# lifunudt/CORB-SLAM

Measured on AMD Instinct MI355X. Metric: stereo frames/sec ORB extract+match, higher is better.
Workload: dtype u8; 1 GPU; configs[1]: ORB extract+match, synthetic 1241x376 stereo stream, 2000 feat/frame, 8 levels x1.2, FAST 20/7; warmup_frames_per_gpu=2560, batches_in_flight=1, distinct_frames=64, parallelism=1 client per GPU, replicas (no collective), inputs=resident in HBM

## Files before the change

### corb-slam_amd/csrc/corb_internal.h

```cpp
#pragma once
#include <hip/hip_runtime.h>
#include <stdint.h>
#include <stddef.h>
#include "../../include/corb_accel.h"

#include <stdlib.h>
#ifdef CORB_DEV
static inline const char* corb_dev_env(const char* name) { return getenv(name); }
#else
static inline const char* corb_dev_env(const char*) { return nullptr; }
#endif

#define CORB_MAX_LEVELS 16
#define CORB_EDGE_THRESHOLD 19
#define CORB_MIN_BORDER 16
#define CORB_HALF_PATCH 15
#define CORB_PATCH_SIZE 31
#define CORB_TH_HIGH 100
#define CORB_TH_LOW 50
#define CORB_HISTO_LENGTH 30

struct CorbLevel {
    int w, h, pitch;
    int plane_off;
    int nCols, nRows, wCell, hCell;
    int maxBX, maxBY;
    int cell_base;
    int cell_cap;
    int cand_base;
    int cand_cap;
    int quota;
    int kp_base, kp_cap;
    int nIni;
    int node_cap;
    int blur_tile_base, blur_tiles_x, blur_tiles_y;
    int resize_tab_off;
    int resize_rec_off;
    float scale;
    float hX;
    int patch_size;
};

#define CORB_BLUR_T 64
#define CORB_MAX_PARTS 4

struct CorbOrbParams {
    int nlevels, n_images;
    int img_base;
    int ini_th, min_th;
    int cells_per_image, cand_per_image, kp_per_image, out_cap;
    int blur_tiles_per_image;
    int node_cap_max, ncell_max;
    int fast_tp, fast_th;
    int pyr_strips;
    short pyr_r0[8][CORB_MAX_LEVELS], pyr_r1[8][CORB_MAX_LEVELS];
    int pyr_ctiles;
    short pyr_g0[8][CORB_MAX_LEVELS], pyr_g1[8][CORB_MAX_LEVELS];
    size_t arena_per_image;
    uint8_t* pyr;
    uint8_t* blur;
    int* cell_count;
    uint32_t* cand;
    uint32_t* keys;
    uint16_t* key_node;
    uint32_t* kp;
    int* kp_count;
    const short* resize_tab;
    const int2* resize_rec;
    CorbKeyPoint* out_kp;
    uint8_t* out_desc;
    int* out_count;
    int* status;
    CorbLevel lv[CORB_MAX_LEVELS];
};

struct CorbStereoParams {
    int n_frames, nlevels;
    int frame_base;
    float bf, mb;
    float scale[CORB_MAX_LEVELS], inv_scale[CORB_MAX_LEVELS];
    int rows0;
    float* u_right;
    float* depth;
    int* sad;
    int* n_matched;
    int* row_off;
    int2* row_idx;
    int row_cap;
    int2* left_range;
};

#ifdef __HIPCC__
__device__ __forceinline__ void corb_xcd_remap(int& unit, int& img)
{
    const unsigned nx = gridDim.x, nimg = gridDim.y;
    const unsigned B = blockIdx.x + nx * blockIdx.y;
    const unsigned g = B / (8u * nx), r = B - g * 8u * nx;
    const unsigned in_group = min(8u, nimg - 8u * g);
    img = (int)(8u * g + r % in_group);
    unit = (int)(r / in_group);
}
#endif

struct CorbStereoDeviceFrame { const CorbKeyPoint* kp; const uint8_t* desc; const float* u_right; const float* depth; const int* count; int cap; hipStream_t stream; int device; };
struct CorbStereo;
int corb_stereo_device_frame(CorbStereo* h, int frame, CorbStereoDeviceFrame* out);
struct CorbRgbd;
int corb_rgbd_device_frame(CorbRgbd* h, int frame, CorbStereoDeviceFrame* out);

struct CorbProfiler;
void corb_orb_device_init();
void corb_launch_ingest(const uint8_t* stage, int w, int h, int n_images, uint8_t* plane, int pitch, size_t image_stride, hipStream_t stream);
void corb_launch_stereo_pack(const CorbOrbParams& p, const CorbStereoParams& s, int frame_base, int n_frames, uint8_t* out, const CorbStereoFrameLayout& lay, hipStream_t stream, struct CorbProfiler* prof);
void corb_launch_orb_pipeline(const CorbOrbParams& p, int img_base, int n_images, size_t octree_lds, hipStream_t stream, CorbProfiler* prof, hipEvent_t after_fast = nullptr);
void corb_launch_candidates(const CorbOrbParams* dp, int img, int level, CorbKeyPoint* out, int cap, int* n_out, hipStream_t stream);
void corb_launch_stereo(const CorbOrbParams& p, const CorbStereoParams& s, int frame_base, int n_frames, hipStream_t stream, CorbProfiler* prof);
size_t corb_octree_lds_bytes(int node_cap_max, int ncell_max);

#ifdef __HIPCC__
#include <hip/hip_ext.h>
#define CORB_LAUNCH(prof, name, kernel, grid, block, lds, stream, ...) do { \
    if ((prof) && (prof)->enabled) { hipEvent_t ea_, eb_; (prof)->pair(name, &ea_, &eb_); hipExtLaunchKernelGGL(kernel, grid, block, (std::uint32_t)(lds), stream, ea_, eb_, 0, __VA_ARGS__); } \
    else hipLaunchKernelGGL(kernel, grid, block, lds, stream, __VA_ARGS__); } while (0)
#endif
#include <vector>
#include <string>
struct CorbProfiler {
    bool enabled = false;
    bool serial = false;
    struct Rec { int name_id; hipEvent_t a, b; };
    std::vector<std::string> names;
    std::vector<Rec> recs;
    std::vector<hipEvent_t> pool;
    int name_id(const char* n) { for (size_t i = 0; i < names.size(); i++) if (names[i] == n) return (int)i; names.push_back(n); return (int)names.size() - 1; }
    void reserve(size_t n) { while (pool.size() < n) { hipEvent_t e; if (hipEventCreate(&e) != hipSuccess) break; pool.push_back(e); } }
    hipEvent_t get() { if (!pool.empty()) { hipEvent_t e = pool.back(); pool.pop_back(); return e; } hipEvent_t e; (void)hipEventCreate(&e); return e; }
    void pair(const char* n, hipEvent_t* a, hipEvent_t* b) { Rec r; r.name_id = name_id(n); r.a = get(); r.b = get(); recs.push_back(r); *a = r.a; *b = r.b; }
    ~CorbProfiler() { for (auto& r : recs) { (void)hipEventDestroy(r.a); (void)hipEventDestroy(r.b); } for (auto e : pool) (void)hipEventDestroy(e); }
};
```

### corb-slam_amd/csrc/corb_orb.cpp

```cpp
#include "corb_internal.h"
#include "orb_handle.h"
#include <cmath>
#include <cfloat>
#include <cstdio>
#include <cstdarg>
#include <cstring>
#include <mutex>
#include <map>
#include <vector>

static thread_local char g_err[512] = "";
void corb_set_error(const char* fmt, ...)
{
    va_list ap; va_start(ap, fmt); vsnprintf(g_err, sizeof(g_err), fmt, ap); va_end(ap);
}
extern "C" const char* corb_last_error(void) { return g_err; }
extern "C" int corb_version(void) { return 100; }
extern "C" int corb_abi_version(void) { return CORB_ABI_VERSION; }
extern "C" int corb_device_count(void)
{
    int n = 0;
    if (hipGetDeviceCount(&n) != hipSuccess) return 0;
    return n;
}
// ... 67 lines not shown
extern "C" int corb_orb_create(const CorbOrbConfig* cfg, CorbOrb** out)
{
    if (!cfg || !out) { corb_set_error("null argument"); return CORB_ERR_ARG; }
    *out = nullptr;
    if (cfg->nlevels < 1 || cfg->nlevels > CORB_MAX_LEVELS || cfg->nfeatures < 1 || cfg->max_images < 1 ||
        cfg->width < 1 || cfg->height < 1 || cfg->width > 4000 || cfg->height > 4000 || !(cfg->scale_factor > 1.0f) ||
        cfg->min_th_fast < 1 || cfg->ini_th_fast < cfg->min_th_fast || cfg->ini_th_fast > 255) {
        corb_set_error("invalid CorbOrbConfig"); return CORB_ERR_ARG;
    }
    int rc = corb_select_device(cfg->device);
    if (rc != CORB_OK) return rc;
    CorbOrb* h = new CorbOrb();
    h->cfg = *cfg;
    const int nl = cfg->nlevels;
    h->scale[0] = 1.0f; h->sigma2[0] = 1.0f;
    for (int i = 1; i < nl; i++) { h->scale[i] = h->scale[i - 1] * cfg->scale_factor; h->sigma2[i] = h->scale[i] * h->scale[i]; }
    for (int i = 0; i < nl; i++) { h->inv_scale[i] = 1.0f / h->scale[i]; h->inv_sigma2[i] = 1.0f / h->sigma2[i]; }
    {
        float factor = 1.0f / cfg->scale_factor;
        float nDesired = cfg->nfeatures * (1 - factor) / (1 - (float)pow((double)factor, (double)nl));
        int sum = 0;
        for (int level = 0; level < nl - 1; level++) { h->quota[level] = cv_round(nDesired); sum += h->quota[level]; nDesired *= factor; }
        h->quota[nl - 1] = std::max(cfg->nfeatures - sum, 0);
        int v, v0, vmax = cv_floor(CORB_HALF_PATCH * sqrtf(2.f) / 2 + 1), vmin = cv_ceil(CORB_HALF_PATCH * sqrtf(2.f) / 2);
        const double hp2 = CORB_HALF_PATCH * CORB_HALF_PATCH;
        for (v = 0; v <= vmax; ++v) h->umax[v] = cv_round(sqrt(hp2 - v * v));
        for (v = CORB_HALF_PATCH, v0 = 0; v >= vmin; --v) { while (h->umax[v0] == h->umax[v0 + 1]) ++v0; h->umax[v] = v0; ++v0; }
        static const int expect[16] = {15, 15, 15, 15, 14, 14, 14, 13, 13, 12, 11, 10, 9, 8, 6, 3};
        for (int i = 0; i < 16; i++) if (h->umax[i] != expect[i]) { corb_set_error("umax table mismatch"); delete h; return CORB_ERR_ARG; }
    }
    CorbOrbParams& p = h->p;
    memset(&p, 0, sizeof(p));
    p.nlevels = nl; p.n_images = cfg->max_images; p.ini_th = cfg->ini_th_fast; p.min_th = cfg->min_th_fast;
    size_t arena = 0; int cells = 0, cands = 0, kps = 0, tiles = 0, tab_off = 0, rec_off = 0;
    for (int l = 0; l < nl; l++) {
        CorbLevel& L = p.lv[l];
        L.w = cv_round((float)cfg->width * h->inv_scale[l]);
        L.h = cv_round((float)cfg->height * h->inv_scale[l]);
        L.pitch = (L.w + 63) & ~63;
        L.plane_off = (int)arena;
        arena += ((size_t)L.pitch * L.h + 255) & ~(size_t)255;
        L.maxBX = L.w - CORB_EDGE_THRESHOLD + 3; L.maxBY = L.h - CORB_EDGE_THRESHOLD + 3;
        const float width = (float)(L.maxBX - CORB_MIN_BORDER), height = (float)(L.maxBY - CORB_MIN_BORDER);
        L.nCols = (int)(width / 30.f); L.nRows = (int)(height / 30.f);
        if (L.nCols < 1 || L.nRows < 1) { corb_set_error("level %d (%dx%d) too small for the 30-px FAST grid", l, L.w, L.h); delete h; return CORB_ERR_ARG; }
        L.wCell = (int)ceilf(width / L.nCols); L.hCell = (int)ceilf(height / L.nRows);
        if (L.wCell > 64 || L.hCell > 64) { corb_set_error("FAST cell %dx%d exceeds the LDS tile", L.wCell, L.hCell); delete h; return CORB_ERR_ARG; }
        L.cell_base = cells; cells += L.nCols * L.nRows;
        L.cell_cap = ((L.wCell + 1) / 2) * ((L.hCell + 1) / 2);
        L.cand_base = cands; L.cand_cap = L.nCols * L.nRows * L.cell_cap; cands += L.cand_cap;
        L.quota = h->quota[l];
        int nIni = (int)roundf(width / height);
        if (nIni < 1) nIni = 1;
        L.nIni = nIni;
        L.hX = width / nIni;
        L.node_cap = ((std::max(L.quota + 3, 4 * nIni) + 1) + 3) & ~3;
        L.kp_base = kps; L.kp_cap = L.node_cap; kps += L.kp_cap;
        L.blur_tiles_x = (L.w + 3) / 4; L.blur_tiles_y = (L.h + 31) / 32;
        L.blur_tile_base = tiles; tiles += (L.blur_tiles_x * L.blur_tiles_y + CORB_BLUR_T - 1) / CORB_BLUR_T;
        L.resize_tab_off = tab_off; tab_off += 3 * L.w + 4 * L.h;
        L.resize_rec_off = rec_off; rec_off += ((L.w + 3) & ~3) + L.h + 4;
        L.scale = h->scale[l];
        L.patch_size = (int)(CORB_PATCH_SIZE * h->scale[l]);
        p.node_cap_max = std::max(p.node_cap_max, L.node_cap);
        p.ncell_max = std::max(p.ncell_max, L.nCols * L.nRows);
        p.fast_tp = std::max(p.fast_tp, 4 * ((L.wCell + 3) / 4) + 8);
        p.fast_th = std::max(p.fast_th, L.hCell + 6);
    }
    p.cells_per_image = cells; p.cand_per_image = cands; p.kp_per_image = kps; p.out_cap = kps;
    p.blur_tiles_per_image = tiles; p.arena_per_image = arena;
    h->octree_lds = corb_octree_lds_bytes(p.node_cap_max, p.ncell_max);
    if (h->octree_lds > 160 * 1024) { corb_set_error("quadtree needs %zu B of LDS (> 160 KiB): nfeatures too large", h->octree_lds); delete h; return CORB_ERR_ARG; }
    if (p.node_cap_max > 65535) { corb_set_error("nfeatures too large"); delete h; return CORB_ERR_ARG; }
    const size_t NI = (size_t)cfg->max_images;
    short* d_tab = nullptr;
#define DA(ptr, n) do { rc = dalloc(h, &(ptr), (n)); if (rc != CORB_OK) { corb_orb_destroy(h); return rc; } } while (0)
    DA(p.pyr, NI * arena); DA(p.blur, NI * arena);
    DA(p.cell_count, NI * cells); DA(p.cand, NI * cands); DA(p.keys, NI * cands); DA(p.key_node, NI * cands);
    DA(p.kp, NI * kps); DA(p.kp_count, NI * CORB_MAX_LEVELS);
    DA(p.out_kp, NI * p.out_cap); DA(p.out_desc, NI * p.out_cap * 32); DA(p.out_count, NI); DA(p.status, NI);
    DA(d_tab, (size_t)tab_off);
    int2* d_rec = nullptr;
    DA(d_rec, (size_t)rec_off + 4);
    DA(h->dp, 1);
#undef DA
    p.resize_tab = d_tab;
    p.resize_rec = d_rec;
    {
        std::vector<short> tab(tab_off);
        for (int l = 1; l < nl; l++) build_resize_tables(p.lv[l - 1].w, p.lv[l - 1].h, p.lv[l].w, p.lv[l].h, tab.data() + p.lv[l].resize_tab_off);
        std::vector<int2> rec((size_t)rec_off + 4, make_int2(0, 0));
        for (int l = 1; l < nl; l++) {
            const short* tl = tab.data() + p.lv[l].resize_tab_off; const int w = p.lv[l].w, hh = p.lv[l].h;
            int2* xr = rec.data() + p.lv[l].resize_rec_off; int2* yr = xr + ((w + 3) & ~3);
            for (int x = 0; x < ((w + 3) & ~3); x++) { const int xc = std::min(x, w - 1); xr[x] = make_int2(tl[xc], (int)(unsigned short)tl[w + xc] | ((int)(unsigned short)tl[2 * w + xc] << 16)); }
            const short* ys0 = tl + 3 * w; const short* ys1 = ys0 + hh; const short* yb0 = ys1 + hh; const short* yb1 = yb0 + hh;
            for (int y = 0; y < hh; y++) yr[y] = make_int2((int)(unsigned short)ys0[y] | ((int)(unsigned short)ys1[y] << 16), (int)(unsigned short)yb0[y] | ((int)(unsigned short)yb1[y] << 16));
        }
        if (hipMemcpy(d_rec, rec.data(), rec.size() * sizeof(int2), hipMemcpyHostToDevice) != hipSuccess) { corb_set_error("resize record upload failed"); corb_orb_destroy(h); return CORB_ERR_HIP; }
        const int S = 4;
        p.pyr_strips = (nl > 1 && p.lv[nl - 1].h >= 4 * S) ? S : 0;
        for (int s = 0; s < p.pyr_strips; s++) {
            int lo = 0, hi = 0;
            for (int l = nl - 1; l >= 1; l--) {
                const int blo = (int)((long long)s * p.lv[l].h / S), bhi = (int)((long long)(s + 1) * p.lv[l].h / S);
                if (l == nl - 1) { lo = blo; hi = bhi; }
                else {
                    const short* tl = tab.data() + p.lv[l + 1].resize_tab_off;
                    const short* ys0 = tl + 3 * p.lv[l + 1].w; const short* ys1 = ys0 + p.lv[l + 1].h;
                    const int clo = ys0[lo], chi = ys1[hi - 1] + 1;
                    lo = std::min(blo, clo); hi = std::max(bhi, chi);
                }
                p.pyr_r0[s][l] = (short)lo; p.pyr_r1[s][l] = (short)hi;
            }
        }
        const int C = 4;
        p.pyr_ctiles = (p.pyr_strips > 0 && p.lv[nl - 1].w >= 16 * C) ? C : 1;
        for (int c = 0; c < p.pyr_ctiles; c++) {
            int lo = 0, hi = 0;
            for (int l = nl - 1; l >= 1; l--) {
                const int ng = (p.lv[l].w + 3) / 4;
                const int blo = (int)((long long)c * ng / p.pyr_ctiles), bhi = (int)((long long)(c + 1) * ng / p.pyr_ctiles);
                if (l == nl - 1) { lo = blo; hi = bhi; }
                else {
                    const short* xofs = tab.data() + p.lv[l + 1].resize_tab_off;
                    const int wn = p.lv[l + 1].w, x_first = std::min(4 * lo, wn - 1), x_last = std::min(4 * hi, wn) - 1;
                    const int clo = xofs[x_first] / 4, chi = std::min(xofs[x_last] + 1, p.lv[l].w - 1) / 4 + 1;
                    lo = std::min(blo, clo); hi = std::max(bhi, chi);
                }
                p.pyr_g0[c][l] = (short)lo; p.pyr_g1[c][l] = (short)hi;
            }
        }
        if (hipMemcpy(d_tab, tab.data(), tab.size() * sizeof(short), hipMemcpyHostToDevice) != hipSuccess ||
            hipMemcpy(h->dp, &p, sizeof(p), hipMemcpyHostToDevice) != hipSuccess ||
            hipMemset(p.status, 0, NI * sizeof(int)) != hipSuccess || hipMemset(p.out_count, 0, NI * sizeof(int)) != hipSuccess ||
            hipMemset(p.pyr, 0, NI * arena) != hipSuccess || hipMemset(p.blur, 0, NI * arena) != hipSuccess ||
            hipStreamCreateWithFlags(&h->stream, hipStreamNonBlocking) != hipSuccess ||
            hipHostMalloc((void**)&h->h_status, NI * sizeof(int)) != hipSuccess ||
            hipHostMalloc((void**)&h->h_count, NI * sizeof(int)) != hipSuccess ||
            hipMalloc((void**)&h->d_stage, (size_t)cfg->width * cfg->height + 256) != hipSuccess ||
            hipHostMalloc((void**)&h->h_img, (size_t)cfg->width * cfg->height) != hipSuccess ||
            hipHostMalloc((void**)&h->h_kp, (size_t)p.out_cap * sizeof(CorbKeyPoint)) != hipSuccess ||
            hipHostMalloc((void**)&h->h_desc, (size_t)p.out_cap * 32) != hipSuccess ||
            hipHostMalloc((void**)&h->h_f32, (size_t)p.out_cap * 2 * sizeof(float)) != hipSuccess ||
            hipHostMalloc((void**)&h->h_misc, 8 * sizeof(int)) != hipSuccess) {
            corb_set_error("device initialisation failed: %s", hipGetErrorString(hipGetLastError()));
            corb_orb_destroy(h); return CORB_ERR_HIP;
        }
    }
    if (const char* e = getenv("CORB_PARTS")) h->parts = std::max(1, std::min(CORB_MAX_PARTS, atoi(e)));
    for (int i = 0; i < CORB_MAX_PARTS; i++)
        if (hipEventCreateWithFlags(&h->ev_stage[i], hipEventDisableTiming) != hipSuccess) { corb_set_error("event creation failed: %s", hipGetErrorString(hipGetLastError())); corb_orb_destroy(h); return CORB_ERR_HIP; }
    *out = h;
    return CORB_OK;
}

extern "C" void corb_orb_destroy(CorbOrb* h)
{
    if (!h) return;
    (void)hipSetDevice(h->cfg.device);
    if (h->stream) { (void)hipStreamSynchronize(h->stream); (void)hipStreamDestroy(h->stream); }
    for (int i = 0; i < CORB_MAX_PARTS - 1; i++) {
        if (h->side[i]) { (void)hipStreamSynchronize(h->side[i]); (void)hipStreamDestroy(h->side[i]); }
        if (h->ev_done[i]) (void)hipEventDestroy(h->ev_done[i]);
    }
    for (int i = 0; i < CORB_MAX_PARTS; i++) if (h->ev_stage[i]) (void)hipEventDestroy(h->ev_stage[i]);
    for (void* ptr : h->allocs) (void)hipFree(ptr);
    if (h->h_status) (void)hipHostFree(h->h_status);
    if (h->h_count) (void)hipHostFree(h->h_count);
    if (h->d_stage) (void)hipFree(h->d_stage);
// ... 448 lines not shown
```

### corb-slam_amd/csrc/orb_kernels.hip

```cpp
#include "corb_internal.h"
#include "lane_exchange.h"
#include <atomic>
#include <cstring>
#include <cstdlib>
#include "brief_pattern.h"

#define WAVE 64

struct CorbDescribeTab { uint4 patb[64]; };
__device__ CorbDescribeTab g_dsc_tab;


#define RS_ROWS 8
__global__ __launch_bounds__(256) void orb_resize_kernel(const CorbOrbParams p, int level)
{
    const CorbLevel& D = p.lv[level];
    const CorbLevel& S = p.lv[level - 1];
    const int img = p.img_base + blockIdx.z;
    const int x4 = (blockIdx.x * 64 + threadIdx.x) * 4;
    const int yb = (blockIdx.y * 4 + threadIdx.y) * RS_ROWS;
    if (x4 >= D.w || yb >= D.h) return;
    const short* tab = p.resize_tab + D.resize_tab_off;
    const short* xofs = tab, * xa0 = tab + D.w, * xa1 = tab + 2 * D.w;
    const short* ys0 = tab + 3 * D.w, * ys1 = ys0 + D.h, * yb0 = ys1 + D.h, * yb1 = yb0 + D.h;
// ... 105 lines not shown
                s1b |= (uint32_t)(ob < 8 ? ob : 0x0c) << (8 * k); s2b |= (uint32_t)(ob < 8 ? k : ob - 4) << (8 * k);
            }
            const bool patch_a = __any(wide && sx[3] - bx >= 8), patch_b = __any(wide && sx1[3] - bx >= 8);
            if (wide) {
                auto fetch = [&](const int2 yr, uint32_t (&w)[6], uint32_t& bb) {
                    const uint32_t* q0 = reinterpret_cast<const uint32_t*>(src + (uint32_t)(__mul24(yr.x & 0xFFFF, S.pitch) + bx));
                    const uint32_t* q1 = reinterpret_cast<const uint32_t*>(src + (uint32_t)(__mul24(yr.x >> 16, S.pitch) + bx));
                    w[0] = q0[0]; w[1] = q0[1]; w[2] = q0[2]; w[3] = q1[0]; w[4] = q1[1]; w[5] = q1[2];
                    bb = (uint32_t)yr.y;
                };
                auto emit = [&](int y, const uint32_t (&w)[6], uint32_t bb) {
                    const uint32_t b0 = bb & 0xFFFFu, b1 = bb >> 16;
                    uint32_t P0 = __builtin_amdgcn_perm(w[1], w[0], s1a), P1 = __builtin_amdgcn_perm(w[1], w[0], s1b);
                    uint32_t Q0 = __builtin_amdgcn_perm(w[4], w[3], s1a), Q1 = __builtin_amdgcn_perm(w[4], w[3], s1b);
                    if (patch_a) { P0 = __builtin_amdgcn_perm(w[2], P0, s2a); Q0 = __builtin_amdgcn_perm(w[5], Q0, s2a); }
                    if (patch_b) { P1 = __builtin_amdgcn_perm(w[2], P1, s2b); Q1 = __builtin_amdgcn_perm(w[5], Q1, s2b); }
                    uint32_t packed = 0;
                    pyr_px<0>(packed, P0, P1, Q0, Q1, A0[0], A1[0], b0, b1, two);
                    pyr_px<1>(packed, P0, P1, Q0, Q1, A0[1], A1[1], b0, b1, two);
                    pyr_px<2>(packed, P0, P1, Q0, Q1, A0[2], A1[2], b0, b1, two);
                    pyr_px<3>(packed, P0, P1, Q0, Q1, A0[3], A1[3], b0, b1, two);
                    uint8_t* dst = dstp + (uint32_t)(__mul24(y, D.pitch) + x4);
                    if (nvalid == 4) *reinterpret_cast<uint32_t*>(dst) = packed;
                    else for (int k = 0; k < nvalid; k++) dst[k] = (uint8_t)(packed >> (8 * k));
                };
                int y = r0 + ty;
                const int ylast = max(r1 - 1, 0);
                int2 ya = yrec[min(y, ylast)], yb = yrec[min(y + RY, ylast)];
                int2 yc = yrec[min(y + 2 * RY, ylast)], yd = yrec[min(y + 3 * RY, ylast)];
#pragma unroll 1
                for (; y + 3 * RY < r1; y += 4 * RY) {
                    uint32_t wa[6], wb[6], wc[6], wd[6], ba, bb, bc, bd;
                    fetch(ya, wa, ba); fetch(yb, wb, bb); fetch(yc, wc, bc); fetch(yd, wd, bd);
                    const int2 na = yrec[min(y + 4 * RY, ylast)], nb = yrec[min(y + 5 * RY, ylast)], nc = yrec[min(y + 6 * RY, ylast)], nd = yrec[min(y + 7 * RY, ylast)];
                    emit(y, wa, ba); emit(y + RY, wb, bb); emit(y + 2 * RY, wc, bc); emit(y + 3 * RY, wd, bd);
                    ya = na; yb = nb; yc = nc; yd = nd;
                }
                if (y + RY < r1) {
                    uint32_t wa[6], wb[6], ba, bb;
                    fetch(ya, wa, ba); fetch(yb, wb, bb);
                    emit(y, wa, ba); emit(y + RY, wb, bb);
                    y += 2 * RY; ya = yc; yb = yd;
                }
                if (y < r1) { uint32_t wa[6], ba; fetch(ya, wa, ba); emit(y, wa, ba); }
            } else {
#pragma unroll 1
                for (int y = r0 + ty; y < r1; y += RY) {
                    const int2 yr = yrec[y];
                    const uint8_t* S0 = src + (uint32_t)__mul24(yr.x & 0xFFFF, S.pitch);
                    const uint8_t* S1 = src + (uint32_t)__mul24(yr.x >> 16, S.pitch);
                    const uint32_t b0 = yr.y & 0xFFFF, b1 = (uint32_t)yr.y >> 16;
                    uint32_t packed = 0;
#pragma unroll
                    for (int k = 0; k < 4; k++) {
                        const uint32_t d0 = mad24u(S0[sx[k]], A0[k] >> 12, mul24u(S0[sx1[k]], A1[k] >> 12));
                        const uint32_t d1 = mad24u(S1[sx[k]], A0[k] >> 12, mul24u(S1[sx1[k]], A1[k] >> 12));
                        const uint32_t v = (((mul24u(b0, d0 >> 4) >> 16) + (mul24u(b1, d1 >> 4) >> 16) + 2u) >> 2) & 0xFFu;
                        packed |= v << (8 * k);
                    }
                    uint8_t* dst = dstp + (uint32_t)(__mul24(y, D.pitch) + x4);
                    if (nvalid == 4) *reinterpret_cast<uint32_t*>(dst) = packed;
                    else for (int k = 0; k < nvalid; k++) dst[k] = (uint8_t)(packed >> (8 * k));
                }
            }
        }
        __threadfence_block();
        __syncthreads();
    }
}


__device__ __forceinline__ uint32_t pk_min3(uint32_t a, uint32_t b, uint32_t c)
{ uint32_t d; asm("v_pk_minimum3_f16 %0, %1, %2, %3" : "=v"(d) : "v"(a), "v"(b), "v"(c)); return d; }
__device__ __forceinline__ uint32_t pk_max3(uint32_t a, uint32_t b, uint32_t c)
{ uint32_t d; asm("v_pk_maximum3_f16 %0, %1, %2, %3" : "=v"(d) : "v"(a), "v"(b), "v"(c)); return d; }
template <int K> __device__ __forceinline__ uint32_t pk_pair(const uint32_t (&w)[3])
{
    static_assert(K >= 0 && K <= 10, "window");
    if constexpr (K <= 6) return __builtin_amdgcn_perm(w[1], w[0], 0x0c000c00u | (uint32_t)K | ((uint32_t)(K + 1) << 16));
    else return __builtin_amdgcn_perm(w[2], w[1], 0x0c000c00u | (uint32_t)(K - 4) | ((uint32_t)(K - 3) << 16));
}
typedef short corb_short2 __attribute__((ext_vector_type(2)));

__device__ __forceinline__ uint32_t fast_ring_score(const uint32_t (&v)[16], uint32_t cpk)
{
    uint32_t lo3[16], hi3[16];
#pragma unroll
    for (int i = 0; i < 16; i++) {
        lo3[i] = pk_min3(v[i], v[(i + 1) & 15], v[(i + 2) & 15]);
        hi3[i] = pk_max3(v[i], v[(i + 1) & 15], v[(i + 2) & 15]);
    }
    uint32_t lo9[16], hi9[16];
#pragma unroll
    for (int i = 0; i < 16; i++) {
        lo9[i] = pk_min3(lo3[i], lo3[(i + 3) & 15], lo3[(i + 6) & 15]);
        hi9[i] = pk_max3(hi3[i], hi3[(i + 3) & 15], hi3[(i + 6) & 15]);
    }
    uint32_t b5[5], d5[5];
#pragma unroll
    for (int i = 0; i < 5; i++) { b5[i] = pk_max3(lo9[3 * i], lo9[3 * i + 1], lo9[3 * i + 2]); d5[i] = pk_min3(hi9[3 * i], hi9[3 * i + 1], hi9[3 * i + 2]); }
    const uint32_t B = pk_max3(pk_max3(b5[0], b5[1], b5[2]), pk_max3(b5[3], b5[4], lo9[15]), b5[0]);
    const uint32_t D = pk_min3(pk_min3(d5[0], d5[1], d5[2]), pk_min3(d5[3], d5[4], hi9[15]), d5[0]);
    const corb_short2 c = __builtin_bit_cast(corb_short2, cpk);
    const corb_short2 s = __builtin_elementwise_max(__builtin_bit_cast(corb_short2, B) - c, c - __builtin_bit_cast(corb_short2, D)) - (short)1;
    return __builtin_bit_cast(uint32_t, s);
}

template <int J> __device__ __forceinline__ uint32_t fast_pair_score(const uint32_t (&R)[7][3], uint32_t th2)
{
    constexpr int C = 4 + 2 * J;
    uint32_t v[16];
    v[0] = pk_pair<C>(R[6]);      v[1] = pk_pair<C + 1>(R[6]);  v[2] = pk_pair<C + 2>(R[5]);  v[3] = pk_pair<C + 3>(R[4]);
    v[4] = pk_pair<C + 3>(R[3]);  v[5] = pk_pair<C + 3>(R[2]);  v[6] = pk_pair<C + 2>(R[1]);  v[7] = pk_pair<C + 1>(R[0]);
    v[8] = pk_pair<C>(R[0]);      v[9] = pk_pair<C - 1>(R[0]);  v[10] = pk_pair<C - 2>(R[1]); v[11] = pk_pair<C - 3>(R[2]);
    v[12] = pk_pair<C - 3>(R[3]); v[13] = pk_pair<C - 3>(R[4]); v[14] = pk_pair<C - 2>(R[5]); v[15] = pk_pair<C - 1>(R[6]);
    const corb_short2 s = __builtin_bit_cast(corb_short2, fast_ring_score(v, pk_pair<C>(R[3])));
    const corb_short2 keep = s >= __builtin_bit_cast(corb_short2, th2);
    return __builtin_bit_cast(uint32_t, (corb_short2)(s & keep));
}

template <int J> __device__ __forceinline__ uint32_t fast_compass(const uint32_t (&R0)[3], const uint32_t (&R3)[3], const uint32_t (&R6)[3])
{
    constexpr int C = 4 + 2 * J;
    const uint32_t v0 = pk_pair<C>(R6), v4 = pk_pair<C + 3>(R3), v8 = pk_pair<C>(R0), v12 = pk_pair<C - 3>(R3), cpk = pk_pair<C>(R3);
    const uint32_t m = pk_min3(pk_max3(v0, v8, v8), pk_max3(v4, v12, v12), pk_max3(v4, v12, v12));
    const uint32_t n = pk_max3(pk_min3(v0, v8, v8), pk_min3(v4, v12, v12), pk_min3(v4, v12, v12));
    const corb_short2 c = __builtin_bit_cast(corb_short2, cpk);
    return __builtin_bit_cast(uint32_t, __builtin_elementwise_max(__builtin_bit_cast(corb_short2, m) - c, c - __builtin_bit_cast(corb_short2, n)));
}
__device__ __forceinline__ int mbcnt64(unsigned long long m) { return (int)__builtin_amdgcn_mbcnt_hi((uint32_t)(m >> 32), __builtin_amdgcn_mbcnt_lo((uint32_t)m, 0u)); }

#define FAST_LIST_CAP 512
__device__ __forceinline__ int wave_incl_scan(int v)
{
    v += __builtin_amdgcn_update_dpp(0, v, 0x111, 0xf, 0xf, true);
    v += __builtin_amdgcn_update_dpp(0, v, 0x112, 0xf, 0xf, true);
    v += __builtin_amdgcn_update_dpp(0, v, 0x114, 0xf, 0xf, true);
    v += __builtin_amdgcn_update_dpp(0, v, 0x118, 0xf, 0xf, true);
    v += __builtin_amdgcn_update_dpp(0, v, 0x142, 0xa, 0xf, true);
    v += __builtin_amdgcn_update_dpp(0, v, 0x143, 0xc, 0xf, true);
    return v;
}
template <int TP>
__global__ __launch_bounds__(64) void orb_fast_kernel(const CorbOrbParams p)
{
    constexpr int P = TP / 4;
    extern __shared__ __attribute__((aligned(16))) uint8_t fast_smem[];
    __shared__ uint16_t plist[FAST_LIST_CAP];
    uint32_t* tile = reinterpret_cast<uint32_t*>(fast_smem);
    uint32_t* sc = tile + P * p.fast_th;
    uint32_t (*rowm)[2] = reinterpret_cast<uint32_t (*)[2]>(sc + P * p.fast_th);
    const int nrowm = p.fast_th - 6;
    uint8_t* scb = reinterpret_cast<uint8_t*>(sc);
    int cell, img; corb_xcd_remap(cell, img); img += p.img_base;
    const int lane = threadIdx.x;
    int level = 0;
    for (int l = 1; l < p.nlevels; l++) if (cell >= p.lv[l].cell_base) level = l;
    const CorbLevel& L = p.lv[level];
    const int c = cell - L.cell_base;
    const int ci = c / L.nCols, cj = c - ci * L.nCols;
    const int iniX = CORB_MIN_BORDER + cj * L.wCell, iniY = CORB_MIN_BORDER + ci * L.hCell;
    const int maxX = min(iniX + L.wCell + 6, L.maxBX), maxY = min(iniY + L.hCell + 6, L.maxBY);
    const int cw = maxX - iniX, ch = maxY - iniY;
    int* out_count = p.cell_count + (size_t)img * p.cells_per_image + cell;
    if (cw < 7 || ch < 7) { if (lane == 0) *out_count = 0; return; }
    const int iw = cw - 6, ih = ch - 6;
    {
        const int gx0 = iniX - 1, a = gx0 & 3;
        const uint8_t* src = p.pyr + (size_t)img * p.arena_per_image + L.plane_off + (size_t)iniY * L.pitch + (gx0 - a);
        const int jlast = (a + cw) >> 2;
        const int r0 = lane / P, wc = lane - r0 * P;
        constexpr int RPI = 64 / P;
        if (r0 < RPI) {
            const int j0 = min(wc, jlast), j1 = min(wc + 1, jlast);
            for (int y = r0; y < ch; y += 4 * RPI) {
                uint32_t w0[4], w1[4];
#pragma unroll
                for (int k = 0; k < 4; k++) {
                    const uint32_t* g = reinterpret_cast<const uint32_t*>(src + (uint32_t)__mul24(min(y + k * RPI, ch - 1), L.pitch));
                    w0[k] = g[j0]; w1[k] = g[j1];
                }
#pragma unroll
                for (int k = 0; k < 4; k++)
                    if (y + k * RPI < ch) { tile[(y + k * RPI) * P + wc] = __builtin_amdgcn_alignbyte(w1[k], w0[k], (uint32_t)a); sc[(y + k * RPI) * P + wc] = 0u; }
            }
        }
    }
    __syncthreads();
    const int ng = (iw + 3) >> 2;
    const int rstep = 64 / ng;
    const int r = (lane * ((65536 + ng - 1) / ng)) >> 16, g = lane - r * ng;
    const bool active = r < rstep;
    const int nvalid = min(4, iw - 4 * g);
    const uint32_t smask0 = nvalid >= 2 ? 0x80008000u : nvalid == 1 ? 0x00008000u : 0u, smask1 = nvalid >= 4 ? 0x80008000u : nvalid == 3 ? 0x00008000u : 0u;
    unsigned long long mine = 0;
    for (int pass = 0; pass < 2; pass++) {
        const int th = pass == 0 ? p.ini_th : p.min_th;
        const uint32_t th2 = (uint32_t)th * 0x00010001u;
        if (lane < nrowm) { rowm[lane][0] = 0u; rowm[lane][1] = 0u; }
        int y0 = 3, nbatch = 0, base = 0, nscore = 0;
        while (y0 < ch - 3) {
            nbatch++;
            base = 0;
            for (; y0 < ch - 3 && base + 128 <= FAST_LIST_CAP; y0 += rstep) {
                const int y = y0 + r;
                bool hit0 = false, hit1 = false;
                if (active && y < ch - 3) {
                    const uint32_t* t = tile + y * P + g;
                    uint32_t R0[3], R3[3], R6[3];
#pragma unroll
                    for (int k = 0; k < 3; k++) { R0[k] = t[-3 * P + k]; R3[k] = t[k]; R6[k] = t[3 * P + k]; }
                    const uint32_t d0 = __builtin_bit_cast(uint32_t, (corb_short2)(__builtin_bit_cast(corb_short2, th2) - __builtin_bit_cast(corb_short2, fast_compass<0>(R0, R3, R6))));
                    const uint32_t d1 = __builtin_bit_cast(uint32_t, (corb_short2)(__builtin_bit_cast(corb_short2, th2) - __builtin_bit_cast(corb_short2, fast_compass<1>(R0, R3, R6))));
                    hit0 = (d0 & smask0) != 0u; hit1 = (d1 & smask1) != 0u;
                }
                const unsigned long long b0 = __ballot(hit0), b1 = __ballot(hit1);
                const int n0 = __popcll(b0);
                const uint32_t ent = (uint32_t)((y << 6) | (g << 1));
                if (hit0) plist[base + mbcnt64(b0)] = (uint16_t)ent;
                if (hit1) plist[base + n0 + mbcnt64(b1)] = (uint16_t)(ent | 1u);
                base += n0 + __popcll(b1);
            }
            __syncthreads();
            nscore = 0;
            for (int i0 = 0; i0 < base; i0 += 64) {
                const int i = i0 + lane;
                bool has = false;
                uint32_t e = 0;
                if (i < base) {
                e = plist[i];
                const int y = e >> 6, ge = (e >> 1) & 31;
                const uint32_t sh = (e & 1u) * 2u;
                const uint32_t* t = tile + y * P + ge;
                uint32_t R[7][3];
#pragma unroll
                for (int dy = 0; dy < 7; dy++) {
                    const uint32_t w0 = t[(dy - 3) * P], w1 = t[(dy - 3) * P + 1], w2 = t[(dy - 3) * P + 2];
                    R[dy][0] = __builtin_amdgcn_alignbyte(w1, w0, sh); R[dy][1] = __builtin_amdgcn_alignbyte(w2, w1, sh); R[dy][2] = __builtin_amdgcn_alignbyte(0u, w2, sh);
                }
                const uint32_t s0 = fast_pair_score<0>(R, th2);
                const int px = 4 * ge + (int)sh;
                uint32_t v = __builtin_amdgcn_perm(0u, s0, 0x0c0c0200u);
                if (px + 1 >= iw) v &= 0xFFu;
                reinterpret_cast<uint16_t*>(scb)[(y * TP + 4 + px) >> 1] = (uint16_t)v;
                has = v != 0u;
                }
                const unsigned long long bs = __ballot(has);
                if (has) plist[nscore + mbcnt64(bs)] = (uint16_t)e;
                nscore += __popcll(bs);
            }
            __syncthreads();
        }
        auto nms_group = [&](int y, int ge) {
            const uint32_t* t = sc + y * P + ge;
            if (t[1] == 0u) return;
            uint32_t S[3][3];
#pragma unroll
            for (int dy = 0; dy < 3; dy++)
#pragma unroll
                for (int k = 0; k < 3; k++) S[dy][k] = t[(dy - 1) * P + k];
            uint32_t bits = 0;
#pragma unroll
            for (int j = 0; j < 2; j++) {
                uint32_t ctr, nb;
                if (j == 0) {
                    ctr = pk_pair<4>(S[1]);
                    nb = pk_max3(pk_max3(pk_pair<3>(S[0]), pk_pair<4>(S[0]), pk_pair<5>(S[0])),
                                 pk_max3(pk_pair<3>(S[2]), pk_pair<4>(S[2]), pk_pair<5>(S[2])),
                                 pk_max3(pk_pair<3>(S[1]), pk_pair<5>(S[1]), pk_pair<5>(S[1])));
                } else {
                    ctr = pk_pair<6>(S[1]);
                    nb = pk_max3(pk_max3(pk_pair<5>(S[0]), pk_pair<6>(S[0]), pk_pair<7>(S[0])),
                                 pk_max3(pk_pair<5>(S[2]), pk_pair<6>(S[2]), pk_pair<7>(S[2])),
                                 pk_max3(pk_pair<5>(S[1]), pk_pair<7>(S[1]), pk_pair<7>(S[1])));
                }
                const uint32_t dm = __builtin_bit_cast(uint32_t, (corb_short2)(__builtin_bit_cast(corb_short2, nb) - __builtin_bit_cast(corb_short2, ctr)));
                bits |= (((dm >> 15) & 1u) | ((dm >> 30) & 2u)) << (2 * j);
            }
            if (bits) atomicOr(&rowm[y - 3][ge >> 3], bits << (4 * (ge & 7)));
        };
        if (nbatch == 1) {
            for (int i = lane; i < nscore; i += 64) {
                const uint32_t e = plist[i];
                const int y = e >> 6, ge = (e >> 1) & 31;
                const uint32_t sh = (e & 1u) * 2u;
                const uint32_t* t = sc + y * P + ge;
                uint32_t S[3][3];
#pragma unroll
                for (int dy = 0; dy < 3; dy++) {
                    const uint32_t w0 = t[(dy - 1) * P], w1 = t[(dy - 1) * P + 1], w2 = t[(dy - 1) * P + 2];
                    S[dy][0] = __builtin_amdgcn_alignbyte(w1, w0, sh); S[dy][1] = __builtin_amdgcn_alignbyte(w2, w1, sh); S[dy][2] = 0u;
                }
                const uint32_t ctr = pk_pair<4>(S[1]);
                const uint32_t nb = pk_max3(pk_max3(pk_pair<3>(S[0]), pk_pair<4>(S[0]), pk_pair<5>(S[0])),
                                            pk_max3(pk_pair<3>(S[2]), pk_pair<4>(S[2]), pk_pair<5>(S[2])),
                                            pk_max3(pk_pair<3>(S[1]), pk_pair<5>(S[1]), pk_pair<5>(S[1])));
                const uint32_t dm = __builtin_bit_cast(uint32_t, (corb_short2)(__builtin_bit_cast(corb_short2, nb) - __builtin_bit_cast(corb_short2, ctr)));
                const uint32_t bits = ((dm >> 15) & 1u) | ((dm >> 30) & 2u);
                if (bits) atomicOr(&rowm[y - 3][ge >> 3], bits << (4 * (ge & 7) + sh));
            }
        } else if (active) {
            for (int y = 3 + r; y < ch - 3; y += rstep) nms_group(y, g);
        }
        __syncthreads();
        mine = lane < ih ? ((unsigned long long)rowm[lane][1] << 32) | rowm[lane][0] : 0ull;
        if (__any(mine != 0ull)) break;
        __syncthreads();
    }
    unsigned long long mask = mine;
    const int cnt = __popcll(mask);
    const int incl = wave_incl_scan(cnt);
    const int total = __builtin_amdgcn_readlane(incl, 63);
    uint32_t* out = p.cand + (size_t)img * p.cand_per_image + L.cand_base + (size_t)c * L.cell_cap;
    int off = incl - cnt;
    while (mask) {
        const int x = __ffsll((long long)mask) - 1;
        mask &= mask - 1;
        if (off < L.cell_cap)
            out[off] = (uint32_t)(iniX + x + 3 - CORB_MIN_BORDER) | ((uint32_t)(iniY + lane + 3 - CORB_MIN_BORDER) << 12) |
                       ((uint32_t)scb[(lane + 3) * TP + x + 4] << 24);
        off++;
    }
    if (lane == 0) { *out_count = min(total, L.cell_cap); if (total > L.cell_cap) p.status[img] = CORB_ERR_OVERFLOW; }
}

#define BL_ROWS 32
#define BL_CHUNK 8
__device__ __forceinline__ int reflect101(int v, int n) { if (v < 0) v = -v; if (v >= n) v = 2 * n - 2 - v; return min(max(v, 0), n - 1); }
#define BLW4(b0, b1, b2, b3) ((uint32_t)(b0) | ((uint32_t)(b1) << 8) | ((uint32_t)(b2) << 16) | ((uint32_t)(b3) << 24))
#define BLW2(lo, hi) ((uint32_t)(lo) | ((uint32_t)(hi) << 16))
typedef unsigned short bl_us2 __attribute__((ext_vector_type(2)));
__device__ __forceinline__ uint32_t bl_dot2(uint32_t a, uint32_t w, uint32_t c)
{ return __builtin_amdgcn_udot2(__builtin_bit_cast(bl_us2, a), __builtin_bit_cast(bl_us2, w), c, false); }
__device__ __forceinline__ uint32_t bl_sat_pk(uint32_t a) { uint32_t d; asm("v_sat_pk_u8_i16 %0, %1" : "=v"(d) : "v"(a)); return d; }

template <bool INTERIOR>
__device__ __forceinline__ void blur_strip(const uint8_t* __restrict__ src, uint8_t* __restrict__ dst, int x, int y0, int y1, int h, int pitch, int wimg)
{
    const int xl = max(x - 4, 0);
    auto load_chunk = [&](uint32_t (&W)[BL_CHUNK][3], int first_row) {
        if (__all(first_row >= 0 && first_row + BL_CHUNK <= h)) {
            const uint32_t o0 = (uint32_t)__mul24(first_row, pitch) + (uint32_t)xl;
#pragma unroll
            for (int i = 0; i < BL_CHUNK; i++) {
                const uint32_t* row = reinterpret_cast<const uint32_t*>(src + (o0 + (uint32_t)(i * pitch)));
                W[i][0] = row[0]; W[i][1] = row[1]; W[i][2] = row[2];
            }
            return;
        }
#pragma unroll
        for (int i = 0; i < BL_CHUNK; i++) {
            const uint32_t off = (uint32_t)__mul24(reflect101(first_row + i, h), pitch) + (uint32_t)xl;
            const uint32_t* row = reinterpret_cast<const uint32_t*>(src + off);
            W[i][0] = row[0]; W[i][1] = row[1]; W[i][2] = row[2];
        }
    };
    uint32_t selA[3] = {0, 0, 0}, selB[3] = {0, 0, 0};
    if (!INTERIOR) {
#pragma unroll
        for (int k = 0; k < 12; k++) {
            const uint32_t q = (uint32_t)min(max(reflect101(x - 4 + k, wimg) - xl, 0), 11);
            selA[k >> 2] |= (q < 8 ? q : 0x0cu) << ((k & 3) * 8);
            selB[k >> 2] |= (q < 8 ? 0x0cu : q - 8) << ((k & 3) * 8);
        }
    }
    auto hsum = [&](const uint32_t (&w)[3], uint32_t (&o)[4]) {
        uint32_t w0 = w[0], w1 = w[1], w2 = w[2];
        if (!INTERIOR) {
            const uint32_t v0 = __builtin_amdgcn_perm(w[1], w[0], selA[0]) | __builtin_amdgcn_perm(0u, w[2], selB[0]);
            const uint32_t v1 = __builtin_amdgcn_perm(w[1], w[0], selA[1]) | __builtin_amdgcn_perm(0u, w[2], selB[1]);
            const uint32_t v2 = __builtin_amdgcn_perm(w[1], w[0], selA[2]) | __builtin_amdgcn_perm(0u, w[2], selB[2]);
            w0 = v0; w1 = v1; w2 = v2;
        }
        o[0] = __builtin_amdgcn_udot4(w1, BLW4(55, 49, 34, 18), __builtin_amdgcn_udot4(w0, BLW4(0, 18, 34, 49), 0u, false), false);
        o[1] = __builtin_amdgcn_udot4(w2, BLW4(18, 0, 0, 0), __builtin_amdgcn_udot4(w1, BLW4(49, 55, 49, 34), __builtin_amdgcn_udot4(w0, BLW4(0, 0, 18, 34), 0u, false), false), false);
        o[2] = __builtin_amdgcn_udot4(w2, BLW4(34, 18, 0, 0), __builtin_amdgcn_udot4(w1, BLW4(34, 49, 55, 49), __builtin_amdgcn_udot4(w0, BLW4(0, 0, 0, 18), 0u, false), false), false);
        o[3] = __builtin_amdgcn_udot4(w2, BLW4(49, 34, 18, 0), __builtin_amdgcn_udot4(w1, BLW4(18, 34, 49, 55), 0u, false), false);
    };
    auto hpair = [&](const uint32_t (&wa)[3], const uint32_t (&wb)[3], uint32_t (&q)[4]) {
        uint32_t a[4], b[4];
        hsum(wa, a); hsum(wb, b);
#pragma unroll
        for (int k = 0; k < 4; k++) q[k] = a[k] | (b[k] << 16);
    };
    const uint32_t bias = 1u << 15;
    auto emit = [&](const uint32_t (&acc)[4], int oy) {
        if (oy >= y1) return;
        const uint32_t s01 = bl_sat_pk(__builtin_amdgcn_perm(acc[1], acc[0], 0x07060302u));
        const uint32_t s23 = bl_sat_pk(__builtin_amdgcn_perm(acc[3], acc[2], 0x07060302u));
        const uint32_t packed = __builtin_amdgcn_perm(s23, s01, 0x05040100u);
        uint8_t* d = dst + ((uint32_t)__mul24(oy, pitch) + (uint32_t)x);
        if (INTERIOR || x + 4 <= wimg) *reinterpret_cast<uint32_t*>(d) = packed;
        else {
            if (x < wimg) d[0] = (uint8_t)packed;
            if (x + 1 < wimg) d[1] = (uint8_t)(packed >> 8);
            if (x + 2 < wimg) d[2] = (uint8_t)(packed >> 16);
        }
    };
    uint32_t Q[4][4];
    uint32_t A[BL_CHUNK][3];
    load_chunk(A, y0 - 3);
    hpair(A[0], A[1], Q[0]); hpair(A[2], A[3], Q[1]); hpair(A[4], A[5], Q[2]);
// ... 728 lines not shown
```

Measured before the change: 107,100 stereo frames/s.

## Precompute FAST cell geometry table and prune the dark-arc chain with a cardinal pre-test

Cell geometry (source offset, origin, dimensions, lane mapping constants) is now computed once on the host into a device table and loaded as a single uint4 per block. This replaces the per-block level search, divisions and min/max arithmetic. The FAST score is also restructured. A test on the four cardinal pixels classifies each pixel pair as bright-only, dark-only or both. Dark-only pairs are turned into bright by XOR-flipping the ring values, and the second min/max arc chain runs only when some lane in the wave needs both polarities. This cuts ALU work in the FAST pass, but adds a wave-divergent branch and extra bit tricks that must stay numerically equivalent to the old score.

```diff
diff --git a/corb-slam_amd/csrc/corb_internal.h b/corb-slam_amd/csrc/corb_internal.h
--- a/corb-slam_amd/csrc/corb_internal.h
+++ b/corb-slam_amd/csrc/corb_internal.h
@@ -41,6 +41,13 @@
     int patch_size;
 };
 
+struct CorbFastCell {
+    uint32_t src_off;
+    uint32_t org;
+    uint32_t dim;
+    uint32_t lane;
+};
+
 #define CORB_BLUR_T 64
 #define CORB_MAX_PARTS 4
 
@@ -67,6 +74,7 @@
     int* kp_count;
     const short* resize_tab;
     const int2* resize_rec;
+    const CorbFastCell* fast_cells;
     CorbKeyPoint* out_kp;
     uint8_t* out_desc;
     int* out_count;
diff --git a/corb-slam_amd/csrc/corb_orb.cpp b/corb-slam_amd/csrc/corb_orb.cpp
--- a/corb-slam_amd/csrc/corb_orb.cpp
+++ b/corb-slam_amd/csrc/corb_orb.cpp
@@ -173,10 +173,32 @@
     DA(d_tab, (size_t)tab_off);
     int2* d_rec = nullptr;
     DA(d_rec, (size_t)rec_off + 4);
+    CorbFastCell* d_cells = nullptr;
+    DA(d_cells, (size_t)cells);
     DA(h->dp, 1);
 #undef DA
     p.resize_tab = d_tab;
     p.resize_rec = d_rec;
+    p.fast_cells = d_cells;
+    {
+        std::vector<CorbFastCell> fc((size_t)cells);
+        for (int l = 0; l < nl; l++) {
+            const CorbLevel& L = p.lv[l];
+            for (int c = 0; c < L.nCols * L.nRows; c++) {
+                const int ci = c / L.nCols, cj = c - ci * L.nCols;
+                const int iniX = CORB_MIN_BORDER + cj * L.wCell, iniY = CORB_MIN_BORDER + ci * L.hCell;
+                const int cw = std::min(iniX + L.wCell + 6, L.maxBX) - iniX, ch = std::min(iniY + L.hCell + 6, L.maxBY) - iniY;
+                CorbFastCell& f = fc[(size_t)L.cell_base + c];
+                f.org = (uint32_t)(iniX + 3 - CORB_MIN_BORDER) | ((uint32_t)(iniY + 3 - CORB_MIN_BORDER) << 12) | ((uint32_t)l << 24);
+                if (cw < 7 || ch < 7) { f.src_off = 0; f.org |= 0x80000000u; f.dim = 0; f.lane = 0; continue; }
+                const int gx0 = iniX - 1, a = gx0 & 3, ng = (cw - 6 + 3) >> 2;
+                f.src_off = (uint32_t)L.plane_off + (uint32_t)iniY * (uint32_t)L.pitch + (uint32_t)(gx0 - a);
+                f.dim = (uint32_t)cw | ((uint32_t)ch << 8) | ((uint32_t)(64 / ng) << 16) | ((uint32_t)ng << 24);
+                f.lane = (uint32_t)((65536 + ng - 1) / ng) | ((uint32_t)((a + cw) >> 2) << 20);
+            }
+        }
+        if (hipMemcpy(d_cells, fc.data(), fc.size() * sizeof(CorbFastCell), hipMemcpyHostToDevice) != hipSuccess) { corb_set_error("FAST cell table upload failed"); corb_orb_destroy(h); return CORB_ERR_HIP; }
+    }
     {
         std::vector<short> tab(tab_off);
         for (int l = 1; l < nl; l++) build_resize_tables(p.lv[l - 1].w, p.lv[l - 1].h, p.lv[l].w, p.lv[l].h, tab.data() + p.lv[l].resize_tab_off);
diff --git a/corb-slam_amd/csrc/orb_kernels.hip b/corb-slam_amd/csrc/orb_kernels.hip
--- a/corb-slam_amd/csrc/orb_kernels.hip
+++ b/corb-slam_amd/csrc/orb_kernels.hip
@@ -211,31 +211,21 @@
 }
 typedef short corb_short2 __attribute__((ext_vector_type(2)));
 
-__device__ __forceinline__ uint32_t fast_ring_score(const uint32_t (&v)[16], uint32_t cpk)
-{
-    uint32_t lo3[16], hi3[16];
-#pragma unroll
-    for (int i = 0; i < 16; i++) {
-        lo3[i] = pk_min3(v[i], v[(i + 1) & 15], v[(i + 2) & 15]);
-        hi3[i] = pk_max3(v[i], v[(i + 1) & 15], v[(i + 2) & 15]);
-    }
-    uint32_t lo9[16], hi9[16];
-#pragma unroll
-    for (int i = 0; i < 16; i++) {
-        lo9[i] = pk_min3(lo3[i], lo3[(i + 3) & 15], lo3[(i + 6) & 15]);
-        hi9[i] = pk_max3(hi3[i], hi3[(i + 3) & 15], hi3[(i + 6) & 15]);
-    }
-    uint32_t b5[5], d5[5];
-#pragma unroll
-    for (int i = 0; i < 5; i++) { b5[i] = pk_max3(lo9[3 * i], lo9[3 * i + 1], lo9[3 * i + 2]); d5[i] = pk_min3(hi9[3 * i], hi9[3 * i + 1], hi9[3 * i + 2]); }
-    const uint32_t B = pk_max3(pk_max3(b5[0], b5[1], b5[2]), pk_max3(b5[3], b5[4], lo9[15]), b5[0]);
-    const uint32_t D = pk_min3(pk_min3(d5[0], d5[1], d5[2]), pk_min3(d5[3], d5[4], hi9[15]), d5[0]);
-    const corb_short2 c = __builtin_bit_cast(corb_short2, cpk);
-    const corb_short2 s = __builtin_elementwise_max(__builtin_bit_cast(corb_short2, B) - c, c - __builtin_bit_cast(corb_short2, D)) - (short)1;
-    return __builtin_bit_cast(uint32_t, s);
-}
-
-template <int J> __device__ __forceinline__ uint32_t fast_pair_score(const uint32_t (&R)[7][3], uint32_t th2)
+template <bool BRIGHT> __device__ __forceinline__ uint32_t fast_arc_chain(const uint32_t (&v)[16])
+{
+    auto in3 = [](uint32_t a, uint32_t b, uint32_t c) { return BRIGHT ? pk_min3(a, b, c) : pk_max3(a, b, c); };
+    auto out3 = [](uint32_t a, uint32_t b, uint32_t c) { return BRIGHT ? pk_max3(a, b, c) : pk_min3(a, b, c); };
+    uint32_t w3[16], w9[16], r5[5];
+#pragma unroll
+    for (int i = 0; i < 16; i++) w3[i] = in3(v[i], v[(i + 1) & 15], v[(i + 2) & 15]);
+#pragma unroll
+    for (int i = 0; i < 16; i++) w9[i] = in3(w3[i], w3[(i + 3) & 15], w3[(i + 6) & 15]);
+#pragma unroll
+    for (int i = 0; i < 5; i++) r5[i] = out3(w9[3 * i], w9[3 * i + 1], w9[3 * i + 2]);
+    return out3(out3(r5[0], r5[1], r5[2]), out3(r5[3], r5[4], w9[15]), r5[0]);
+}
+
+template <int J> __device__ __forceinline__ uint32_t fast_pair_score(const uint32_t (&R)[7][3], uint32_t th2, uint32_t kb, uint32_t kd)
 {
     constexpr int C = 4 + 2 * J;
     uint32_t v[16];
@@ -243,7 +233,18 @@
     v[4] = pk_pair<C + 3>(R[3]);  v[5] = pk_pair<C + 3>(R[2]);  v[6] = pk_pair<C + 2>(R[1]);  v[7] = pk_pair<C + 1>(R[0]);
     v[8] = pk_pair<C>(R[0]);      v[9] = pk_pair<C - 1>(R[0]);  v[10] = pk_pair<C - 2>(R[1]); v[11] = pk_pair<C - 3>(R[2]);
     v[12] = pk_pair<C - 3>(R[3]); v[13] = pk_pair<C - 3>(R[4]); v[14] = pk_pair<C - 2>(R[5]); v[15] = pk_pair<C - 1>(R[6]);
-    const corb_short2 s = __builtin_bit_cast(corb_short2, fast_ring_score(v, pk_pair<C>(R[3])));
+    const uint32_t cpk = pk_pair<C>(R[3]);
+    const uint32_t e0 = pk_max3(v[0], v[8], v[8]), e1 = pk_max3(v[4], v[12], v[12]), f0 = pk_min3(v[0], v[8], v[8]), f1 = pk_min3(v[4], v[12], v[12]);
+    const uint32_t m = pk_min3(e0, e1, e1), n = pk_max3(f0, f1, f1);
+    const uint32_t nbright = (cpk + kb) - m;
+    const uint32_t dark = ((cpk + kd) - n) & 0x02000200u;
+    const uint32_t donly = dark & nbright, both = dark ^ donly;
+    const uint32_t xm = (donly >> 1) - (donly >> 9);
+#pragma unroll
+    for (int i = 0; i < 16; i++) v[i] ^= xm;
+    const corb_short2 c = __builtin_bit_cast(corb_short2, cpk ^ xm) + (short)1;
+    corb_short2 s = __builtin_bit_cast(corb_short2, fast_arc_chain<true>(v)) - c;
+    if (__any(both != 0u)) s = __builtin_elementwise_max(s, c - (short)2 - __builtin_bit_cast(corb_short2, fast_arc_chain<false>(v)));
     const corb_short2 keep = s >= __builtin_bit_cast(corb_short2, th2);
     return __builtin_bit_cast(uint32_t, (corb_short2)(s & keep));
 }
@@ -283,21 +284,19 @@
     uint8_t* scb = reinterpret_cast<uint8_t*>(sc);
     int cell, img; corb_xcd_remap(cell, img); img += p.img_base;
     const int lane = threadIdx.x;
-    int level = 0;
-    for (int l = 1; l < p.nlevels; l++) if (cell >= p.lv[l].cell_base) level = l;
-    const CorbLevel& L = p.lv[level];
+    uint4 rec = reinterpret_cast<const uint4*>(p.fast_cells)[cell];
+    asm volatile("" : "+s"(rec.x));
+    int* out_count = p.cell_count + (size_t)img * p.cells_per_image + cell;
+    if (rec.y >> 31) { if (lane == 0) *out_count = 0; return; }
+    const CorbLevel& L = p.lv[(rec.y >> 24) & 15u];
     const int c = cell - L.cell_base;
-    const int ci = c / L.nCols, cj = c - ci * L.nCols;
-    const int iniX = CORB_MIN_BORDER + cj * L.wCell, iniY = CORB_MIN_BORDER + ci * L.hCell;
-    const int maxX = min(iniX + L.wCell + 6, L.maxBX), maxY = min(iniY + L.hCell + 6, L.maxBY);
-    const int cw = maxX - iniX, ch = maxY - iniY;
-    int* out_count = p.cell_count + (size_t)img * p.cells_per_image + cell;
-    if (cw < 7 || ch < 7) { if (lane == 0) *out_count = 0; return; }
+    const int ox = (int)(rec.y & 0xFFFu), oy = (int)((rec.y >> 12) & 0xFFFu);
+    const int cw = (int)(rec.z & 0xFFu), ch = (int)((rec.z >> 8) & 0xFFu);
     const int iw = cw - 6, ih = ch - 6;
     {
-        const int gx0 = iniX - 1, a = gx0 & 3;
-        const uint8_t* src = p.pyr + (size_t)img * p.arena_per_image + L.plane_off + (size_t)iniY * L.pitch + (gx0 - a);
-        const int jlast = (a + cw) >> 2;
+        const uint32_t a = (uint32_t)ox & 3u;
+        const uint8_t* src = p.pyr + (size_t)img * p.arena_per_image + rec.x;
+        const int jlast = (int)(rec.w >> 20);
         const int r0 = lane / P, wc = lane - r0 * P;
         constexpr int RPI = 64 / P;
         if (r0 < RPI) {
@@ -311,14 +310,13 @@
                 }
 #pragma unroll
                 for (int k = 0; k < 4; k++)
-                    if (y + k * RPI < ch) { tile[(y + k * RPI) * P + wc] = __builtin_amdgcn_alignbyte(w1[k], w0[k], (uint32_t)a); sc[(y + k * RPI) * P + wc] = 0u; }
+                    if (y + k * RPI < ch) { tile[(y + k * RPI) * P + wc] = __builtin_amdgcn_alignbyte(w1[k], w0[k], a); sc[(y + k * RPI) * P + wc] = 0u; }
             }
         }
     }
     __syncthreads();
-    const int ng = (iw + 3) >> 2;
-    const int rstep = 64 / ng;
-    const int r = (lane * ((65536 + ng - 1) / ng)) >> 16, g = lane - r * ng;
+    const int rstep = (int)((rec.z >> 16) & 0xFFu), ng = (int)(rec.z >> 24);
+    const int r = (int)(((uint32_t)lane * (rec.w & 0xFFFFFu)) >> 16), g = lane - r * ng;
     const bool active = r < rstep;
     const int nvalid = min(4, iw - 4 * g);
     const uint32_t smask0 = nvalid >= 2 ? 0x80008000u : nvalid == 1 ? 0x00008000u : 0u, smask1 = nvalid >= 4 ? 0x80008000u : nvalid == 3 ? 0x00008000u : 0u;
@@ -326,6 +324,7 @@
     for (int pass = 0; pass < 2; pass++) {
         const int th = pass == 0 ? p.ini_th : p.min_th;
         const uint32_t th2 = (uint32_t)th * 0x00010001u;
+        const uint32_t kb = th2 + 0x02000200u, kd = 0x02000200u - th2 - 0x00010001u;
         if (lane < nrowm) { rowm[lane][0] = 0u; rowm[lane][1] = 0u; }
         int y0 = 3, nbatch = 0, base = 0, nscore = 0;
         while (y0 < ch - 3) {
@@ -367,7 +366,7 @@
                     const uint32_t w0 = t[(dy - 3) * P], w1 = t[(dy - 3) * P + 1], w2 = t[(dy - 3) * P + 2];
                     R[dy][0] = __builtin_amdgcn_alignbyte(w1, w0, sh); R[dy][1] = __builtin_amdgcn_alignbyte(w2, w1, sh); R[dy][2] = __builtin_amdgcn_alignbyte(0u, w2, sh);
                 }
-                const uint32_t s0 = fast_pair_score<0>(R, th2);
+                const uint32_t s0 = fast_pair_score<0>(R, th2, kb, kd);
                 const int px = 4 * ge + (int)sh;
                 uint32_t v = __builtin_amdgcn_perm(0u, s0, 0x0c0c0200u);
                 if (px + 1 >= iw) v &= 0xFFu;
@@ -446,7 +445,7 @@
         const int x = __ffsll((long long)mask) - 1;
         mask &= mask - 1;
         if (off < L.cell_cap)
-            out[off] = (uint32_t)(iniX + x + 3 - CORB_MIN_BORDER) | ((uint32_t)(iniY + lane + 3 - CORB_MIN_BORDER) << 12) |
+            out[off] = (uint32_t)(ox + x) | ((uint32_t)(oy + lane) << 12) |
                        ((uint32_t)scb[(lane + 3) * TP + x + 4] << 24);
         off++;
     }
```

Result: faster. 108,600 stereo frames/s (median of 6 runs) (+1.4%).
